# andrewhou1/BlindShadowRemoval

Hardware: AMD Instinct MI355X
Metric: images/sec at 256x256 batch inference (GSC generator forward) (higher is better)
Workload: dtype f32; 1 GPU; BASELINE configs[1]: batch=32 synthetic 256x256x3 per GPU, full GSC generator fp32 (seeded random-init weights in the ckpt-94 variable layout); global_batch=32, height=256, width=256, parallelism=dp1, forwards_in_flight=1, collective=none

## Files before the change

### blindshadowremoval_amd/csrc/bsr_api.hip

```cpp
#include "../../include/bsr_hip.h"

#include <hip/hip_runtime.h>
#include <stdint.h>
#include <stdio.h>
#include <stdlib.h>
#include <string.h>

#include <initializer_list>
#include <string>
#include <type_traits>
#include <unordered_map>
#include <vector>

#include "attention.h"
#include "attention256.h"
#include "attention_h16.h"
#include "conv3_f16.h"
#include "conv_n16.h"
#include "gemm_nloop.h"
#include "glue_kernels.h"
#include "igemm_conv.h"
#include "igemm_h16.h"
#include "png_kernels.h"
#include "prep_kernels.h"
// ... 123 lines not shown
constexpr Variant kTSM16{true, false, 291, 320, 288, 291, 320, 877, 896, 874};
constexpr Variant kRGB{false, true, 99, 128, 96, 513, 544, 0, 0, 0, 256, 3, 192, 256, 544, 128, 32};
constexpr int CS_Y3X = kGSC.cs_y3x;
constexpr int CS_CF = 64;
constexpr int RGB_CS_R = kRGB.cs_r, RGB_CS_A = kRGB.cs_a, RGB_D = kRGB.d, RGB_CS_C3 = kRGB.cs_c3, RGB_CS_C2 = kRGB.cs_c2, RGB_CS_QH = kRGB.cs_qh;

struct Region {
  size_t off, floats;
};
struct Plan {
  size_t x1, c3, c2, xa, t1, t2, y3[6], qkv, att[6], r[6], xh, ybuf, qh, f1, f2, cf, probe, reg32, share, yh, con, total;
  Region zero[8];
  int nzero;
};

Plan make_plan(size_t B, size_t H, size_t W, const Variant& v) {
  Plan p{};
  size_t off = 0;
  auto take = [&](size_t floats, bool keep_zero = false) {
    size_t o = off;
    off += (floats + 63) & ~size_t(63);
    if (keep_zero && floats != 0) p.zero[p.nzero++] = {o, floats};
    return o;
  };
  const size_t px = B * H * W, cells = px / 64;
  const size_t px2 = v.rgb ? 0 : px;
  const size_t px1 = px - px2;
  p.x1 = take(px * 32);
  p.c3 = take(px / 4 * v.cs_c3);
  p.c2 = take(px / 16 * v.cs_c2);
  p.xa = take(cells * v.cs_a, true);
  p.t1 = take(cells * v.d);
  p.t2 = take(cells * v.d);
  for (int i = 0; i < v.nblk; ++i) p.y3[i] = take(cells * v.cs_y3x);
  p.qkv = take(cells * 3 * v.d);
  for (int i = 0; i < v.nblk; ++i) p.att[i] = take(cells * v.d);
  for (int i = 0; i < v.nblk; ++i) p.r[i] = take(cells * (i < 3 ? v.cs_r : v.cs_h), !v.rgb);
  p.xh = take(cells * v.cs_h, true);
  p.ybuf = take(px * v.cs_y);
  p.qh = take(px * v.cs_qh);
  p.f1 = take(px2 / 16 * 128);
  p.f2 = take(px2 / 4 * 96);
  p.cf = take(px2 * CS_CF);
  p.probe = take(px2 / 64 * 2);
  p.reg32 = take(v.tsm ? cells * 4 : 0);
  p.share = take(v.tsm ? cells * 2 * v.c_r : 0);
  p.yh = take(px1 * 3);
  p.con = take(px1 * 3);
  p.total = off;
  return p;
}

}

struct bsr_handle {
  int device = 0;
  float* d_blob = nullptr;
  float* d_wino = nullptr;
  float* d_keys = nullptr;
  float* d_values = nullptr;
  float* att_scratch = nullptr;
  size_t att_scratch_floats = 0;
  std::unordered_map<std::string, LayerW> layers;
  Variant var = kGSC;
  int dtype = BSR_DTYPE_F32;
  float head_bias[2] = {0.f, 0.f};
  const float* tail_w = nullptr;
  const float* clr_gs_w = nullptr;
  float* ws = nullptr;
  size_t ws_floats = 0;
  Plan plan{};
  const float* rgb_tail_w = nullptr;
  const float* rgb_head_b = nullptr;
  int B = 0, H = 0, W = 0;
  bool ran = false;
  bool att_in_lds = false;
  unsigned* range_flag = nullptr;
  bool fuse_heads = true;
  bool conv1_gemm = true;
  bool att_pv1 = false;
  bool conv3_f16 = true;
  bool fuse_attw = true;
  bool wino_conv2 = true;
  bool keys_conv2 = true;
  bool values_conv2 = true;
  bool att_is_o = false;
  bool timing = false;
  std::vector<hipEvent_t> ev;
  std::vector<int> ev_class;
  std::vector<std::string> ev_name;
  size_t ev_used = 0;
};

namespace {

const char* const kRangeMsg =
    "an activation exceeded the fp16 range (|x| >= 65520) in a forward of this 16-bit-mode handle: its outputs are not trustworthy "
    "(inf / NaN where the fp32 path stays finite).  Re-run those inputs on a BSR_DTYPE_F32 handle; bsr_check_range() clears the condition";

constexpr size_t kWinoFloats = 8 * 16 * 128 * 16;
void wino_filter_transform(const float* direct, float* out) {
  static const double G[4][3] = {{1.0, 0.0, 0.0}, {0.5, 0.5, 0.5}, {0.5, -0.5, 0.5}, {0.0, 0.0, 1.0}};
  for (int k = 0; k < 128; ++k)
    for (int n = 0; n < 128; ++n) {
      double t[4][3];
      for (int x = 0; x < 4; ++x)
        for (int b = 0; b < 3; ++b) {
          double acc = 0.0;
          for (int a = 0; a < 3; ++a) acc += G[x][a] * (double)direct[((size_t)((k / 32) * 9 + a * 3 + b) * 128 + n) * 36 + k % 32];
          t[x][b] = acc;
        }
      for (int x = 0; x < 4; ++x)
        for (int y = 0; y < 4; ++y) {
          double acc = 0.0;
          for (int b = 0; b < 3; ++b) acc += t[x][b] * G[y][b];
          out[((size_t)((k / 16) * 16 + 4 * x + y) * 128 + n) * 16 + k % 16] = (float)acc;
        }
    }
}

constexpr int kKeysN = 288 + 256, kKeysNPad = kKeysN + 64, kC3qNPad = 768;
constexpr size_t kKeysFloats = (size_t)4 * kKeysNPad * 36 + kKeysNPad;
void keys_compose(const float* c3q_w, const float* c3q_b, float* out_w, float* out_b) {
  auto src = [&](int k, int n) -> const float& { return c3q_w[((size_t)(k / 32) * kC3qNPad + n) * 36 + k % 32]; };
  memset(out_w, 0, (size_t)4 * kKeysNPad * 36 * sizeof(float));
  memset(out_b, 0, kKeysNPad * sizeof(float));
  for (int ch = 0; ch < 4; ++ch) {
    memcpy(out_w + (size_t)ch * kKeysNPad * 36, c3q_w + (size_t)ch * kC3qNPad * 36, (size_t)288 * 36 * sizeof(float));
    memcpy(out_w + ((size_t)ch * kKeysNPad + 416) * 36, c3q_w + ((size_t)ch * kC3qNPad + 544) * 36, (size_t)128 * 36 * sizeof(float));
  }
  memcpy(out_b, c3q_b, 288 * sizeof(float));
  memcpy(out_b + 416, c3q_b + 544, 128 * sizeof(float));
  for (int m = 0; m < 128; ++m) {
    for (int k = 0; k < 128; ++k) {
      double acc = 0.0;
      for (int c = 0; c < 128; ++c) acc += (double)src(k, 288 + c) * (double)src(m, 416 + c);
      out_w[((size_t)(k / 32) * kKeysNPad + 288 + m) * 36 + k % 32] = (float)acc;
    }
    double acc = 0.0;
    for (int c = 0; c < 128; ++c) acc += (double)c3q_b[288 + c] * (double)src(m, 416 + c);
    out_b[288 + m] = (float)acc;
  }
}

constexpr int kWNPad = 384;
constexpr int kValuesN = 288 + 128, kValuesNPad = kValuesN + 64;
constexpr int kGProbeNPad = 128 + 64;
constexpr size_t kValuesWFloats = (size_t)4 * kWNPad * 36 + kWNPad, kValuesC3qFloats = (size_t)4 * kValuesNPad * 36 + kValuesNPad,
                 kGProbeFloats = (size_t)4 * kGProbeNPad * 36 + kGProbeNPad;
constexpr size_t kValuesFloats = kValuesWFloats + kValuesC3qFloats + kGProbeFloats;
void values_compose(const float* c3q_w, const float* c3q_b, const float* w_w, const float* w_b, float* out_w, float* out_b) {
  auto wg = [&](int k, int c) -> double { return (double)c3q_w[((size_t)(k / 32) * kC3qNPad + 544 + c) * 36 + k % 32]; };
  auto ww = [&](int c, int n) -> double { return (double)w_w[((size_t)(c / 32) * kWNPad + n) * 36 + c % 32]; };
  memset(out_w, 0, (size_t)4 * kWNPad * 36 * sizeof(float));
  for (int n = 0; n < kWNPad; ++n) {
    for (int k = 0; k < 128; ++k) {
      double acc = 0.0;
      for (int c = 0; c < 128; ++c) acc += wg(k, c) * ww(c, n);
      out_w[((size_t)(k / 32) * kWNPad + n) * 36 + k % 32] = (float)acc;
    }
    double acc = (double)w_b[n];
    for (int c = 0; c < 128; ++c) acc += (double)c3q_b[544 + c] * ww(c, n);
    out_b[n] = (float)acc;
  }
}
void values_cut(const float* keys_w, const float* keys_b, const float* c3q_w, const float* c3q_b, float* v_w, float* v_b, float* g_w, float* g_b) {
// ... 136 lines not shown
    if (half_tile) {
      if constexpr (kTrunk) check(bsr::launch_igemm_conv<KH, KW, S, TR, 2, 32, 2, 2, 1, 1, CC, INB>(a, h->B, s), name);
    } else if (!h16)
      check(bsr::launch_igemm_conv<KH, KW, S, TR, 4, 32, 4, 1, 1, NI, CC, INB>(a, h->B, s), name);
    else if (nsplit == 2)
      check(bsr::launch_igemm_h16<KH, KW, S, TR, 4, 32, 4, 1, 1, NI, CCH, INB, 2>(a, h->B, s), name);
    else if constexpr (k33)
      with_io(io, [&](auto io_c) { check(bsr::launch_igemm_h16<KH, KW, S, TR, 4, 32, 4, 1, 1, NI, CCH, INB, 1, io_c.value>(a, h->B, s), name); });
    end();
  }
  bsr::ConvArgs gemm_args(const LayerW& l, const float* in, int in_cs, float* out, int out_cs, int n_store, int act) const {
    bsr::ConvArgs a{};
    a.in = in; a.in_cs = in_cs; a.out = out; a.out_cs = out_cs;
    a.w = l.w; a.bias = l.b; a.nchunk = l.nchunk; a.n_pad = l.n_pad; a.n_store = n_store; a.act = act;
    a.range_flag = h->range_flag;
    return a;
  }
  template <int NI, int NCH, int MINW = 2>
  void gemm(int cls, const char* name, const float* in, int in_cs, size_t pixels, float* out, int out_cs, int n_store, int act,
            const float* res1 = nullptr, int res1_cs = 0, int res1_c = 0,
            float* out2 = nullptr, int out2_cs = 0, int n_split = 0, int n_store1 = 0, const LayerW* image = nullptr, int out2_gap_at = 0,
            int out2_gap = 0) {
    if (rc != BSR_OK) return;
    using C = bsr::GemmNLoopCfg<NI, NCH>;
    LayerW l;
    const int tiles = (n_store + 31) / 32;
    int kNSplit = 2;
    {
      const long long mblocks = (long long)(pixels / C::BM);
      const int want = (int)((2LL * bsr::device_cu_count() + mblocks - 1) / (mblocks > 0 ? mblocks : 1));
      const int most = (tiles + NI - 1) / NI;
      kNSplit = want < 2 ? 2 : (want > most ? most : want);
#ifdef BSR_NL_NSPLIT
      kNSplit = BSR_NL_NSPLIT > most ? most : BSR_NL_NSPLIT;
#endif
    }
    if (image == nullptr) rc = find_layer(h, name, NCH, 1, 36, (tiles + NI - 1) * 32, &l);
    else if (image->nchunk == NCH && image->ldp == 36 && image->n_pad >= (tiles + NI - 1) * 32) l = *image;
    else rc = fail(BSR_ERR_ARG, std::string("layer '") + name + "': the handle's image does not fit the kernel");
    if (rc != BSR_OK) return;
    if (pixels % C::BM != 0) { rc = fail(BSR_ERR_ARG, std::string("layer '") + name + "': pixel count is not a multiple of 128"); return; }
    bsr::ConvArgs a = gemm_args(l, in, in_cs, out, out_cs, n_store, act);
    a.res1 = res1; a.res1_cs = res1_cs; a.res1_c = res1_c;
    a.out2 = out2; a.out2_cs = out2_cs; a.n_split = n_split; a.n_store1 = n_store1; a.out2_gap_at = out2_gap_at; a.out2_gap = out2_gap;
    a.out2_split = (h->dtype != BSR_DTYPE_F32 && out2 != nullptr) ? 1 : 0;
    begin(cls, name);
    if (h->dtype == BSR_DTYPE_F32)
      check(bsr::launch_gemm_nloop<NI, NCH, 0, MINW>(a, pixels, kNSplit, s), name);
    else if constexpr (MINW == 2)
      check(bsr::launch_gemm_nloop<NI, NCH, 2>(a, pixels, kNSplit, s), name);
    else
      rc = fail(BSR_ERR_ARG, std::string("layer '") + name + "': the RGB bottleneck GEMMs are fp32 only");
    end();
  }
  template <int NCH>
  void gemm_all_n(const char* name, const float* in, size_t pixels, float* out) {
    if (rc != BSR_OK) return;
    LayerW l;
    rc = find_layer(h, name, NCH, 1, 36, 128, &l);
    if (rc != BSR_OK) return;
    begin(K_CONV1, name);
    check(bsr::launch_gemm_nloop<4, NCH, 2, 1>(gemm_args(l, in, NCH * 32, out, 128, 128, 1), pixels, 1, s), name);
    end();
  }

  void stem(const float* in, int H, int W, float* out) {
    if (rc != BSR_OK) return;
    LayerW l;
    rc = find_layer(h, "conv1", 1, 7, h->dtype != BSR_DTYPE_F32 ? 36 : 28, 32, &l);
    if (rc != BSR_OK) return;
    bsr::StemArgs a{in, out, l.w, l.b, H, W, 0, 0, 0, h->range_flag};
    begin(K_CONV7, "conv1");
    with_dtype(h->dtype, [&](auto prec, auto half) { check(bsr::launch_stem7<4, prec.value, half.value>(a, h->B, s), "conv1"); });
    end();
  }

  void wino(const char* name, int i, const float* in, int H, int W, float* out, int out_cs = 128) {
    if (rc != BSR_OK) return;
    LayerW l;
    rc = find_layer(h, name, 4, 9, 36, 128, &l);
    if (rc != BSR_OK) return;
    if (H % 4 != 0 || W % 32 != 0) { rc = fail(BSR_ERR_ARG, std::string("layer '") + name + "': feature map is not a multiple of the 4x32 tile"); return; }
    begin(K_CONV3, name);
    check(bsr::launch_wino_conv2(wino_args(in, out, h->d_wino + (size_t)i * kWinoFloats, l.b, H, W, out_cs), h->B, s), name);
    end();
  }

  void conv71(const char* name, const float* in, int in_cs, int k_pad, int H, int W, float* out, int out_cs) {
    if (rc != BSR_OK) return;
    LayerW l;
    rc = find_layer(h, name, k_pad / 32, 7, 36, 32, &l);
    if (rc != BSR_OK) return;
    if (H % 4 != 0 || W % 32 != 0) { rc = fail(BSR_ERR_ARG, std::string("layer '") + name + "': image is not a multiple of the 4x32 tile"); return; }
    bsr::ConvArgs a{};
    a.in = in; a.in_cs = in_cs; a.in_coff = 0; a.H = H; a.W = W;
    a.out = out; a.out_cs = out_cs; a.out_coff = 0; a.Ho = H; a.Wo = W;
    a.w = l.w; a.bias = l.b; a.nchunk = l.nchunk; a.n_pad = l.n_pad; a.n_store = 32;
    a.pad_t = 3; a.pad_l = 0; a.act = 0;
    begin(K_CONV7, name);
    check(bsr::launch_igemm_conv<7, 1, 1, false, 4, 32, 4, 1, 1, 1, 32, 1>(a, h->B, s), name);
    end();
  }

  void heads(const float* y, int H, int W, float* qh, const float* inputs, float* gs, float* mask22, size_t npix) {
    if (rc != BSR_OK) return;
    LayerW l;
    rc = find_layer(h, "heads", 2, 7, 36, 16, &l);
    if (rc != BSR_OK) return;
    if (l.n_pad != 16) { rc = fail(BSR_ERR_BLOB, "layer 'heads' must be packed with n_pad 16"); return; }
    if (H % 8 != 0 || W % 32 != 0) { rc = fail(BSR_ERR_ARG, "layer 'heads': image is not a multiple of its tile"); return; }
    bsr::ConvN16Args a{};
    a.in = y; a.in_cs = 64; a.H = H; a.W = W; a.w = l.w; a.bias = l.b; a.out = qh; a.out_cs = 16; a.act = 0;
    a.pad_t = 3; a.pad_l = 0;
    a.inputs = inputs; a.gs_out = gs; a.mask22 = mask22; a.b_mask = h->head_bias[0]; a.b_con = h->head_bias[1];
    a.range_flag = h->range_flag;
    int resident = 0;
    check(bsr::launch_conv_n16<7, 1, false, false, 2, 0, false, true>(a, h->B, s, &resident), "heads");
    const bool fuse = rc == BSR_OK && h->fuse_heads && bsr::conv_n16_fuse_pays(h->B, H, 8, resident);
    begin(K_CONV7, "heads");
    with_dtype(h->dtype, [&](auto prec, auto half) {
      if (fuse) check(bsr::launch_conv_n16<7, 1, false, false, 2, prec.value, half.value, true>(a, h->B, s), "heads");
      else check(bsr::launch_conv_n16<7, 1, false, false, 2, prec.value, half.value>(a, h->B, s), "heads");
    });
    end();
    if (fuse) return;
    begin(K_GLUE, "heads_post");
    hipLaunchKernelGGL(bsr::heads_post_kernel, dim3((unsigned)((npix + 255) / 256)), dim3(256), 0, s, qh, inputs, h->head_bias[0], h->head_bias[1], gs,
                       mask22, W, npix);
    check(hipGetLastError(), "heads_post");
    end();
  }

  template <int KH, int KW, bool GS, bool TAIL, int RW>
  void conv16(int cls, const char* name, const float* in, int in_cs, int H, int W, float* out, int out_cs, int act, const float* gs,
              const float* inputs, float* con_rgb, float* dif, float* packed = nullptr) {
    if (rc != BSR_OK) return;
    LayerW l;
    rc = find_layer(h, name, 2, KH * KW, 36, 16, &l);
    if (rc != BSR_OK) return;
    if (l.n_pad != 16) { rc = fail(BSR_ERR_BLOB, std::string("layer '") + name + "' must be packed with n_pad 16"); return; }
    bsr::ConvN16Args a{};
    a.in = in; a.in_cs = in_cs; a.H = H; a.W = W; a.w = l.w; a.bias = l.b; a.out = out; a.out_cs = out_cs; a.act = act;
    a.pad_t = (KH - 1) / 2; a.pad_l = (KW - 1) / 2;
    a.gs = gs; a.w_gs = h->clr_gs_w; a.tail_w = h->tail_w; a.inputs = inputs; a.con_rgb = con_rgb; a.dif = dif; a.packed = packed;
    a.range_flag = h->range_flag;
    if (H % (4 * RW) != 0 || W % 32 != 0) { rc = fail(BSR_ERR_ARG, std::string("layer '") + name + "': image is not a multiple of its tile"); return; }
    begin(cls, name);
    with_dtype(h->dtype, [&](auto prec, auto half) { check(bsr::launch_conv_n16<KH, KW, GS, TAIL, RW, prec.value, half.value>(a, h->B, s), name); });
    end();
  }
};

int grow_workspace(bsr_handle* h, size_t floats, bool device_wide, hipStream_t s) {
  if (floats <= h->ws_floats) return BSR_OK;
  if (device_wide) HIP_TRY(hipDeviceSynchronize());
  else HIP_TRY(hipStreamSynchronize(s));
  if (h->ws) HIP_TRY(hipFree(h->ws));
  h->ws = nullptr;
  h->ws_floats = 0;
  HIP_TRY(hipMalloc(reinterpret_cast<void**>(&h->ws), floats * sizeof(float)));
  h->ws_floats = floats;
  h->B = 0;
  h->ran = false;
  if (device_wide) HIP_TRY(hipMemset(h->ws, 0, floats * sizeof(float)));
  else HIP_TRY(hipMemsetAsync(h->ws, 0, floats * sizeof(float), s));
  return BSR_OK;
}

int ensure_workspace(bsr_handle* h, int B, int H, int W, hipStream_t s) {
  const Plan p = make_plan(B, H, W, h->var);
  const bool fresh = p.total > h->ws_floats;
  const int rc = grow_workspace(h, p.total, false, s);
  if (rc != BSR_OK) return rc;
  if (!fresh && (B != h->B || H != h->H || W != h->W)) {
    for (int i = 0; i < p.nzero; ++i) HIP_TRY(hipMemsetAsync(h->ws + p.zero[i].off, 0, p.zero[i].floats * sizeof(float), s));
    h->ran = false;
  }
  h->plan = p;
  h->B = B; h->H = H; h->W = W;
  return BSR_OK;
}

template <typename T>
int read_records(const unsigned char* blob, size_t off, int n, hipStream_t s, std::vector<T>* out) {
  out->resize((size_t)n);
  HIP_TRY(hipMemcpyAsync(out->data(), blob + off, (size_t)n * sizeof(T), hipMemcpyDeviceToHost, s));
  HIP_TRY(hipStreamSynchronize(s));
  return BSR_OK;
}

}

extern "C" {

int bsr_abi_version(void) { return 8; }

#ifndef BSR_SRC_SHA
#define BSR_SRC_SHA "unhashed"
#endif
static const char kSrcShaTag[] = "BSR_SRC_SHA=" BSR_SRC_SHA;
const char* bsr_source_sha(void) { return kSrcShaTag + 12; }

const char* bsr_last_error(void) { return g_last_error.c_str(); }

size_t bsr_workspace_bytes(int B, int H, int W) {
  if (B <= 0 || H <= 0 || W <= 0) return 0;
  return make_plan(B, H, W, kGSC).total * sizeof(float);
}

int bsr_create(bsr_handle** out, int device, const void* packed_weights, size_t nbytes, int dtype) {
  if (out == nullptr || packed_weights == nullptr) return fail(BSR_ERR_ARG, "bsr_create: null argument");
  *out = nullptr;
  if (dtype != BSR_DTYPE_F32 && dtype != BSR_DTYPE_F16 && dtype != BSR_DTYPE_F32X3)
    return fail(BSR_ERR_ARG, "bsr_create: dtype must be BSR_DTYPE_F32, BSR_DTYPE_F16 or BSR_DTYPE_F32X3");
  if (nbytes < sizeof(BlobHeader)) return fail(BSR_ERR_BLOB, "bsr_create: blob shorter than its header");
  const uint8_t* blob = static_cast<const uint8_t*>(packed_weights);
  BlobHeader hd;
  memcpy(&hd, blob, sizeof hd);
  if (hd.magic != kBlobMagic || hd.version != kBlobVersion) return fail(BSR_ERR_BLOB, "bsr_create: bad blob magic/version");
  if ((int)hd.reserved != dtype) return fail(BSR_ERR_BLOB, "bsr_create: the blob was packed for another dtype (pack_generator(weights, dtype) must match bsr_create's dtype)");
  const size_t table_end = sizeof(BlobHeader) + (size_t)hd.n_entries * sizeof(BlobEntry);
  if (table_end > nbytes) return fail(BSR_ERR_BLOB, "bsr_create: blob entry table exceeds blob size");
  DeviceGuard guard(device);
  HIP_TRY(guard.err);
  bsr_handle* h = new bsr_handle();
  h->device = device;
  h->dtype = dtype;
  h->att_pv1 = dtype == BSR_DTYPE_F16;
  const struct { const char* env; bool* on; } switches[] = {{"BSR_FUSE_HEADS", &h->fuse_heads}, {"BSR_FUSE_ATTW", &h->fuse_attw}, {"BSR_CONV3_F16", &h->conv3_f16},
                                                            {"BSR_CONV1_GEMM", &h->conv1_gemm}, {"BSR_WINO_CONV2", &h->wino_conv2},
                                                            {"BSR_KEYS_CONV2", &h->keys_conv2}, {"BSR_VALUES_CONV2", &h->values_conv2}};
  for (const auto& sw : switches)
    if (const char* e_ = getenv(sw.env)) *sw.on = atoi(e_) != 0;
  hipError_t e = hipMalloc(reinterpret_cast<void**>(&h->d_blob), nbytes);
  if (e == hipSuccess) e = hipMemcpy(h->d_blob, blob, nbytes, hipMemcpyHostToDevice);
  if (e != hipSuccess) {
    if (h->d_blob) hipFree(h->d_blob);
    delete h;
    return fail(BSR_ERR_HIP, std::string("bsr_create: weight upload: ") + hipGetErrorString(e));
  }
  for (uint32_t i = 0; i < hd.n_entries; ++i) {
    BlobEntry en;
    memcpy(&en, blob + sizeof(BlobHeader) + (size_t)i * sizeof(BlobEntry), sizeof en);
    en.name[sizeof(en.name) - 1] = 0;
    if (en.offset % 16 != 0 || en.offset + en.nfloats * 4 > nbytes) {
      bsr_destroy(h);
      return fail(BSR_ERR_BLOB, std::string("bsr_create: entry '") + en.name + "' is out of bounds or misaligned");
    }
    std::string nm(en.name);
    const float* dptr = reinterpret_cast<const float*>(reinterpret_cast<const uint8_t*>(h->d_blob) + en.offset);
    if (nm == "heads.bias") {
      if (en.nfloats != 2) { bsr_destroy(h); return fail(BSR_ERR_BLOB, "bsr_create: heads.bias must hold 2 floats"); }
      memcpy(h->head_bias, blob + en.offset, 8);
    } else if (nm == "clr_conv1.gs") {
      if (en.nfloats != 256) { bsr_destroy(h); return fail(BSR_ERR_BLOB, "bsr_create: clr_conv1.gs must hold 16x16 floats"); }
      h->clr_gs_w = dptr;
    } else if (nm == "rgb.tail") {
      if (en.nfloats != 7 * 7 * 3 * 3 + 3) { bsr_destroy(h); return fail(BSR_ERR_BLOB, "bsr_create: rgb.tail must hold 7x7x3x3 + 3 floats"); }
      h->rgb_tail_w = dptr;
    } else if (nm == "rgb.head_bias") {
      if (en.nfloats != 3) { bsr_destroy(h); return fail(BSR_ERR_BLOB, "bsr_create: rgb.head_bias must hold 3 floats"); }
      h->rgb_head_b = dptr;
    } else if (nm == "tail.w") {
      if (en.nfloats != 16 * 16 + 16 + 48 + 3) { bsr_destroy(h); return fail(BSR_ERR_BLOB, "bsr_create: tail.w has the wrong size"); }
      h->tail_w = dptr;
    } else if (nm.size() > 2 && nm.compare(nm.size() - 2, 2, ".w") == 0) {
      LayerW& l = h->layers[nm.substr(0, nm.size() - 2)];
      l.w = dptr;
      l.nchunk = en.dims[0]; l.taps = en.dims[1]; l.n_pad = en.dims[2]; l.ldp = en.dims[3];
      if ((uint64_t)l.nchunk * l.taps * l.n_pad * l.ldp != en.nfloats) {
        bsr_destroy(h);
        return fail(BSR_ERR_BLOB, std::string("bsr_create: entry '") + en.name + "' dims do not match its size");
      }
    } else if (nm.size() > 2 && nm.compare(nm.size() - 2, 2, ".b") == 0) {
      h->layers[nm.substr(0, nm.size() - 2)].b = dptr;
    }
  }
  if (h->layers.count("rgb_head") != 0) {
    if (dtype != BSR_DTYPE_F32) {
      bsr_destroy(h);
      return fail(BSR_ERR_ARG, "bsr_create: these are RGB-baseline weights (model_RGB.py), which run in BSR_DTYPE_F32 only: BSR_DTYPE_F32X3 and BSR_DTYPE_F16 are not provided for them");
    }
    if (h->rgb_tail_w == nullptr || h->rgb_head_b == nullptr) { bsr_destroy(h); return fail(BSR_ERR_BLOB, "bsr_create: RGB blob lacks 'rgb.tail' / 'rgb.head_bias'"); }
    h->var = kRGB;
    *out = h;
    return BSR_OK;
  }
  if (h->tail_w == nullptr || h->clr_gs_w == nullptr) { bsr_destroy(h); return fail(BSR_ERR_BLOB, "bsr_create: blob lacks 'tail.w' / 'clr_conv1.gs'"); }
  if (dtype != BSR_DTYPE_F32) {
    e = hipHostMalloc(reinterpret_cast<void**>(&h->range_flag), 64, hipHostMallocMapped);
    if (e != hipSuccess) { h->range_flag = nullptr; bsr_destroy(h); return fail(BSR_ERR_HIP, std::string("bsr_create: range flag: ") + hipGetErrorString(e)); }
    *h->range_flag = 0u;
  }
  {
    auto it = h->layers.find("res0.conv1");
    if (it == h->layers.end()) { bsr_destroy(h); return fail(BSR_ERR_BLOB, "bsr_create: blob has no 'res0.conv1'"); }
    const int nch = it->second.nchunk;
    if (dtype == BSR_DTYPE_F32) h->var = nch == 13 ? kTSM : kGSC;
    else h->var = nch == 10 ? kTSM16 : kGSC16;
  }
  if (dtype == BSR_DTYPE_F32) {
    std::vector<float> u(6 * kWinoFloats);
    for (int i = 0; i < 6; ++i) {
      char nm[32];
      snprintf(nm, sizeof nm, "res%d.conv2", i);
      LayerW l;
      if (find_layer(h, nm, 4, 9, 36, 128, &l) != BSR_OK || l.n_pad != 128) { bsr_destroy(h); return fail(BSR_ERR_BLOB, std::string("bsr_create: layer '") + nm + "' is not a [4][9][128][36] image"); }
      wino_filter_transform(reinterpret_cast<const float*>(blob + (reinterpret_cast<const uint8_t*>(l.w) - reinterpret_cast<const uint8_t*>(h->d_blob))), u.data() + i * kWinoFloats);
    }
    e = hipMalloc(reinterpret_cast<void**>(&h->d_wino), u.size() * sizeof(float));
    if (e == hipSuccess) e = hipMemcpy(h->d_wino, u.data(), u.size() * sizeof(float), hipMemcpyHostToDevice);
    if (e != hipSuccess) { bsr_destroy(h); return fail(BSR_ERR_HIP, std::string("bsr_create: Winograd weights: ") + hipGetErrorString(e)); }
    std::vector<float> q(6 * kKeysFloats);
// ... 997 lines not shown
size_t bsr_sfw_score_scratch_bytes(int B, int S) { return post_size_ok(B, S) ? (size_t)B * bsr::sfw_item_scratch_bytes(S) : 0; }

int bsr_sfw_score(int device, const float* rows3, int B, int S, float* losses, double* auc, float* pred, float* label, int* status,
                  void* scratch, void* stream) {
  return run_post("bsr_sfw_score", {rows3, losses, auc, pred, label, status, scratch}, B, S, scratch, device, [&] {
    HIP_TRY(bsr::launch_sfw_score(rows3, B, S, losses, auc, pred, label, status, scratch, static_cast<hipStream_t>(stream)));
    return BSR_OK;
  });
}

int bsr_clock_trace(int device, unsigned long long* out, int samples, int spin, const int* stop, int* taken, void* stream) {
  if (out == nullptr || stop == nullptr || taken == nullptr || samples <= 0 || spin < 0) return fail(BSR_ERR_ARG, "bsr_clock_trace: bad argument");
  DeviceGuard guard(device);
  HIP_TRY(guard.err);
  hipLaunchKernelGGL(bsr::clock_trace_kernel, dim3(1), dim3(64), 0, static_cast<hipStream_t>(stream), out, samples, spin, stop, taken);
  HIP_TRY(hipGetLastError());
  return BSR_OK;
}

int bsr_debug_split_qkv(const float* qkv, void* qkv_split, int B, int tokens, void* stream) {
  if (qkv == nullptr || qkv_split == nullptr) return fail(BSR_ERR_ARG, "bsr_debug_split_qkv: null argument");
  if (B <= 0 || tokens <= 0 || tokens % 128 != 0) return fail(BSR_ERR_ARG, "bsr_debug_split_qkv: tokens must be a positive multiple of 128");
  const size_t pairs = (size_t)B * tokens * 192;
  hipLaunchKernelGGL(bsr::a4_split_qkv_kernel, dim3((unsigned)((pairs + 255) / 256)), dim3(256), 0, static_cast<hipStream_t>(stream), qkv,
                     static_cast<char*>(qkv_split), pairs);
  HIP_TRY(hipGetLastError());
  return BSR_OK;
}

int bsr_debug_attention_split(const void* qkv_split, float* y, int B, int tokens, int pv1, void* stream) {
  if (qkv_split == nullptr || y == nullptr) return fail(BSR_ERR_ARG, "bsr_debug_attention_split: null argument");
  if (B <= 0 || tokens <= 0 || tokens % 128 != 0) return fail(BSR_ERR_ARG, "bsr_debug_attention_split: tokens must be a positive multiple of 128");
  HIP_TRY(bsr::launch_nonlocal_attention_h16(static_cast<const float*>(qkv_split), y, B, tokens, static_cast<hipStream_t>(stream), pv1 != 0));
  return BSR_OK;
}

int bsr_debug_attention_dtype(const float* qkv, float* y, int B, int tokens, int dtype, void* stream) {
  if (qkv == nullptr || y == nullptr) return fail(BSR_ERR_ARG, "bsr_debug_attention: null argument");
  if (B <= 0 || tokens <= 0 || tokens % 128 != 0) return fail(BSR_ERR_ARG, "bsr_debug_attention: tokens must be a positive multiple of 128");
  if (dtype == BSR_DTYPE_F32) {
    HIP_TRY(bsr::launch_nonlocal_attention(qkv, y, B, tokens, static_cast<hipStream_t>(stream)));
  } else if (dtype == BSR_DTYPE_F32X3 || dtype == BSR_DTYPE_F16) {
    void* tmp = nullptr;
    HIP_TRY(hipMalloc(&tmp, (size_t)B * tokens * bsr::kA4TokBytes));
    int rc = bsr_debug_split_qkv(qkv, tmp, B, tokens, stream);
    if (rc == BSR_OK) rc = bsr_debug_attention_split(tmp, y, B, tokens, 0, stream);
    hipError_t e = hipStreamSynchronize(static_cast<hipStream_t>(stream));
    hipFree(tmp);
    if (rc != BSR_OK) return rc;
    HIP_TRY(e);
  } else {
    return fail(BSR_ERR_ARG, "bsr_debug_attention: unknown dtype");
  }
  return BSR_OK;
}

int bsr_debug_attention_qw(const float* qkv, float* y, int B, int tokens, int qw, void* stream) {
  if (qkv == nullptr || y == nullptr) return fail(BSR_ERR_ARG, "bsr_debug_attention_qw: null argument");
  if (B <= 0 || tokens <= 0 || tokens % 128 != 0) return fail(BSR_ERR_ARG, "bsr_debug_attention_qw: tokens must be a positive multiple of 128");
  if (qw != 0 && qw != 1 && qw != 2 && qw != 4) return fail(BSR_ERR_ARG, "bsr_debug_attention_qw: qw must be 0 (automatic), 1, 2 or 4 query waves per workgroup");
  HIP_TRY(bsr::launch_nonlocal_attention(qkv, y, B, tokens, static_cast<hipStream_t>(stream), qw));
  return BSR_OK;
}

int bsr_debug_attention_kv1(const float* qkv2, float* y, int B, int tokens, int qw, void* stream) {
  if (qkv2 == nullptr || y == nullptr) return fail(BSR_ERR_ARG, "bsr_debug_attention_kv1: null argument");
  if (B <= 0 || tokens <= 0 || tokens % 128 != 0) return fail(BSR_ERR_ARG, "bsr_debug_attention_kv1: tokens must be a positive multiple of 128");
  if (qw != 0 && qw != 1 && qw != 2 && qw != 4) return fail(BSR_ERR_ARG, "bsr_debug_attention_kv1: qw must be 0 (automatic), 1, 2 or 4 query waves per workgroup");
  HIP_TRY(bsr::launch_nonlocal_attention<true>(qkv2, y, B, tokens, static_cast<hipStream_t>(stream), qw));
  return BSR_OK;
}

int bsr_debug_attention_rgb(const float* qkv, float* y, int B, int tokens, void* stream) {
  if (qkv == nullptr || y == nullptr) return fail(BSR_ERR_ARG, "bsr_debug_attention_rgb: null argument");
  if (B <= 0 || tokens <= 0 || tokens % 32 != 0) return fail(BSR_ERR_ARG, "bsr_debug_attention_rgb: tokens must be a positive multiple of 32");
  HIP_TRY(bsr::launch_nonlocal_attention256(qkv, y, B, tokens, static_cast<hipStream_t>(stream)));
  return BSR_OK;
}

int bsr_debug_wino_conv(const float* x, const float* w, const float* bias, float* y, int B, int H, int W, int nw, void* stream) {
  if (x == nullptr || w == nullptr || bias == nullptr || y == nullptr) return fail(BSR_ERR_ARG, "bsr_debug_wino_conv: null argument");
  if (B <= 0 || H <= 0 || W <= 0 || H % 4 != 0 || W % 32 != 0) return fail(BSR_ERR_ARG, "bsr_debug_wino_conv: H must be a positive multiple of 4 and W of 32");
  if ((long long)B * H * W * 128 * 4 >= (1LL << 31)) return fail(BSR_ERR_ARG, "bsr_debug_wino_conv: tensor too large");
  if (nw != 0 && nw != 2 && nw != 4) return fail(BSR_ERR_ARG, "bsr_debug_wino_conv: nw must be 0 (automatic), 2 or 4 waves per workgroup");
  HIP_TRY(bsr::launch_wino_conv2(wino_args(x, y, w, bias, H, W), B, static_cast<hipStream_t>(stream), nw));
  return BSR_OK;
}

int bsr_debug_wino_filter(const float* direct, float* out) {
  if (direct == nullptr || out == nullptr) return fail(BSR_ERR_ARG, "bsr_debug_wino_filter: null argument");
  wino_filter_transform(direct, out);
  return BSR_OK;
}

int bsr_debug_keys_compose(const float* c3q_w, const float* c3q_b, float* out_w, float* out_b) {
  if (c3q_w == nullptr || c3q_b == nullptr || out_w == nullptr || out_b == nullptr) return fail(BSR_ERR_ARG, "bsr_debug_keys_compose: null argument");
  keys_compose(c3q_w, c3q_b, out_w, out_b);
  return BSR_OK;
}

int bsr_debug_values_compose(const float* c3q_w, const float* c3q_b, const float* w_w, const float* w_b, float* out_w, float* out_b) {
  if (c3q_w == nullptr || c3q_b == nullptr || w_w == nullptr || w_b == nullptr || out_w == nullptr || out_b == nullptr)
    return fail(BSR_ERR_ARG, "bsr_debug_values_compose: null argument");
  values_compose(c3q_w, c3q_b, w_w, w_b, out_w, out_b);
  return BSR_OK;
}

int bsr_debug_attention(const float* qkv, float* y, int B, int tokens, void* stream) {
  return bsr_debug_attention_dtype(qkv, y, B, tokens, BSR_DTYPE_F32, stream);
}

struct ProbeSrc { size_t off; int hh, ww, cs, coff, c; bool half; int derive; };

static int probe_index(const std::string& nm, const char* prefix, int n) {
  const size_t len = strlen(prefix);
  if (nm.size() == len + 1 && nm.compare(0, len, prefix) == 0 && nm[len] >= '0' && nm[len] < '0' + n) return nm[len] - '0';
  return -1;
}

static int probe_src_rgb(const bsr_handle* h, const std::string& nm, ProbeSrc* src) {
  const Plan& p = h->plan;
  const int H = h->H, W = h->W;
  int i;
  if (nm == "x1") *src = {p.x1, H, W, 32, 0, 32};
  else if (nm == "x2") *src = {p.c3, H / 2, W / 2, RGB_CS_C3, 128, 64};
  else if (nm == "x3") *src = {p.c2, H / 4, W / 4, RGB_CS_C2, 192, 64};
  else if (nm == "x0") *src = {p.xa, H / 8, W / 8, RGB_CS_A, 0, 99};
  else if ((i = probe_index(nm, "res", 3)) >= 0) *src = {p.r[i], H / 8, W / 8, RGB_CS_R, 0, 513};
  else if ((i = probe_index(nm, "att", 3)) >= 0) *src = {p.att[i], H / 8, W / 8, RGB_D, 0, RGB_D};
  else if ((i = probe_index(nm, "y3x", 3)) >= 0) *src = {p.y3[i], H / 8, W / 8, RGB_CS_R, 0, 513};
  else if (nm == "up1") *src = {p.c2, H / 4, W / 4, RGB_CS_C2, 0, 192};
  else if (nm == "up2") *src = {p.c3, H / 2, W / 2, RGB_CS_C3, 0, 128};
  else if (nm == "up3") *src = {p.ybuf, H, W, 128, 0, 128};
  else if (nm == "y") *src = {p.yh, H, W, 3, 0, 3};
  else if (nm == "con") *src = {p.con, H, W, 3, 0, 3};
  else return fail(BSR_ERR_STATE, "bsr_probe: unknown probe '" + nm + "' for an RGB handle");
  return BSR_OK;
}

static int probe_src_gsc(const bsr_handle* h, const std::string& nm, ProbeSrc* src) {
  const Plan& p = h->plan;
  const Variant& v = h->var;
  const int H = h->H, W = h->W;
  const bool p16 = h->dtype == BSR_DTYPE_F16;
  int i;
  if (nm == "x1") *src = {p.x1, H, W, 32, 0, 32, p16};
  else if (nm == "x2") *src = {p.c3, H / 2, W / 2, 128, 64, 64, p16};
  else if (nm == "x3") *src = {p.c2, H / 4, W / 4, 160, 96, 64, p16};
  else if (nm == "x0") *src = {p.xa, H / 8, W / 8, v.cs_a, 0, v.c_a};
  else if ((i = probe_index(nm, "res", 6)) >= 0) *src = {p.r[i], H / 8, W / 8, i < 3 ? v.cs_r : v.cs_h, 0, i < 3 ? v.c_r : v.c_h};
  else if ((i = probe_index(nm, "att", 6)) >= 0) {
    if (h->att_in_lds)
      return fail(BSR_ERR_STATE, "bsr_probe: att<i> does not exist for the last forward — attention and the `w` GEMM ran as one launch and the "
                                 "attention output never left LDS (create the handle with BSR_FUSE_ATTW=0 in the environment to probe it)");
    *src = {p.att[i], H / 8, W / 8, 128, 0, 128, false, h->att_is_o ? i + 1 : 0};
  }
  else if ((i = probe_index(nm, "attv", 6)) >= 0) {
    if (!h->att_is_o) return fail(BSR_ERR_STATE, "bsr_probe: attv<i> exists only for a forward with conv2's output as the attention values (fp32, BSR_KEYS_CONV2 and BSR_VALUES_CONV2 on)");
    if (h->att_in_lds)
      return fail(BSR_ERR_STATE, "bsr_probe: attv<i> does not exist for the last forward — attention and the `w` GEMM ran as one launch and the "
                                 "attention output never left LDS (create the handle with BSR_FUSE_ATTW=0 in the environment to probe it)");
    *src = {p.att[i], H / 8, W / 8, 128, 0, 128};
  }
  else if (nm == "qkv") {
    if (h->dtype != BSR_DTYPE_F32) return fail(BSR_ERR_STATE, "bsr_probe: qkv is an fp32 tensor of BSR_DTYPE_F32 handles only");
    const int c = h->att_is_o ? 256 : 384;
    *src = {p.qkv, H / 8, W / 8, c, 0, c};
// ... 95 lines not shown
```

### blindshadowremoval_amd/csrc/wino_conv2.h

```cpp
#pragma once
#include <hip/hip_runtime.h>
#include <stdint.h>

#include "mfma_common.h"

namespace bsr {

struct WinoArgs {
  const float* in;
  float* out;
  const float* w;
  const float* bias;
  int H, W;
  int in_cs, out_cs;
  int tiles_x, tiles_y;
  int act;
};

template <int NW>
struct WinoCfg {
  static constexpr int NT = NW * 64;
  static constexpr int CC = 16;
  static constexpr int LDP = CC + 4;
  static constexpr int K = 128, N = 128, NCHUNK = K / CC;
// ... 121 lines not shown
  for (int i = 0; i < 4; ++i) store_w1(u_n1, w_regs[1], i);
  fetch_w(2, w_regs[1]);
  __syncthreads();

  f32x16 acc[16];
#pragma unroll
  for (int q = 0; q < 16; ++q)
#pragma unroll
    for (int i = 0; i < 16; ++i) acc[q][i] = 0.f;
  acc[5] = bias_tile(h, bias_n);

  const int a_base = r * LDP + 4 * h;
  const int b_base = (wave * 32 + r) * LDP + 4 * h;
  f32x4 af[2], bf[2];
  auto read_frags = [&](int slot, int v_off, int u_off) {
    af[slot] = *reinterpret_cast<const f32x4*>(s_v + a_base + v_off);
    bf[slot] = *reinterpret_cast<const f32x4*>(s_u + b_base + u_off);
  };
  read_frags(0, v_cur, u_cur);

  for (int ch = 0; ch < C::NCHUNK; ++ch) {
    const int ch1 = ch + 1 < C::NCHUNK ? ch + 1 : C::NCHUNK - 1;
#pragma unroll
    for (int s = 0; s < SPC; ++s) {
      const int t = ch * SPC + s;
      fetch_w(t + 3 < NSTEPS ? t + 3 : NSTEPS - 1, w_regs[s & 1]);
      if (s == 0) fetch_in(ch1, d);
      __builtin_amdgcn_sched_barrier(0);
#pragma unroll
      for (int q = 0; q < 4; ++q) {
        const int cur = q & 1, nxt = cur ^ 1;
        const int pl = q >> 1;
        if (q < 3) {
          const int pl1 = (q + 1) >> 1, g1 = (q + 1) & 1;
          read_frags(nxt, v_cur + (2 * s + pl1) * C::V_POS + g1 * 8, u_cur + pl1 * C::U_POS + g1 * 8);
        } else if (s + 1 < SPC) {
          read_frags(nxt, v_cur + (2 * s + 2) * C::V_POS, u_n1);
        } else {
          read_frags(nxt, v_nxt, u_n1);
        }
        store_w1(u_n2, w_regs[(s + 1) & 1], q);
        if (s == SPC - 3) in_rows(d, q);
        if (s == SPC - 2) in_cols_store(v_nxt, d, q);
        __builtin_amdgcn_sched_barrier(0);
#pragma unroll
        for (int j = 0; j < 4; ++j)
          acc[2 * s + pl] = __builtin_amdgcn_mfma_f32_32x32x2f32(af[cur][j], bf[cur][j], acc[2 * s + pl], 0, 0, 0);
        __builtin_amdgcn_sched_barrier(0);
      }
      __syncthreads();
      { const int tu = u_cur; u_cur = u_n1; u_n1 = u_n2; u_n2 = tu; }
      if (s == SPC - 1) { const int tv = v_cur; v_cur = v_nxt; v_nxt = tv; }
    }
  }

  const float alpha = p.act ? kLeakyAlpha : 1.f;
  const unsigned cs4 = (unsigned)p.out_cs * 4u;
  const __amdgpu_buffer_rsrc_t orsrc =
      make_rsrc(p.out + ((size_t)img * p.H * p.W + (size_t)y0 * p.W + x0) * p.out_cs + n0 + wave * 32);
  const unsigned lane_out = (unsigned)(8 * h) * cs4 + (unsigned)r * 4u;
#pragma unroll
  for (int v = 0; v < 16; ++v) {
    float t0[4], t1[4];
#pragma unroll
    for (int nu = 0; nu < 4; ++nu) {
      t0[nu] = (acc[nu][v] + acc[4 + nu][v]) + acc[8 + nu][v];
      t1[nu] = (acc[4 + nu][v] - acc[8 + nu][v]) - acc[12 + nu][v];
    }
    f32x2 y0v = f32x2{(t0[0] + t0[1]) + t0[2], (t0[1] - t0[2]) - t0[3]};
    f32x2 y1v = f32x2{(t1[0] + t1[1]) + t1[2], (t1[1] - t1[2]) - t1[3]};
    const f32x2 s0 = y0v * alpha, s1 = y1v * alpha;
    const int prow = 2 * (v >> 3), pcol = 2 * (8 * ((v >> 2) & 1) + (v & 3));
#pragma unroll
    for (int i = 0; i < 2; ++i)
#pragma unroll
      for (int j = 0; j < 2; ++j) {
        const float x = i ? y1v[j] : y0v[j], ax = i ? s1[j] : s0[j];
        const unsigned soff = (unsigned)((prow + i) * p.W + pcol + j) * cs4;
        __builtin_amdgcn_raw_buffer_store_b32(__float_as_uint(__builtin_amdgcn_fmed3f(x, ax, 3.4028234664e38f)), orsrc, lane_out, soff, 0);
      }
  }
}

inline int wino_conv2_auto_nw(int batch, int H, int W) {
  const long long tiles = (long long)batch * (H / 4) * (W / 32);
  return 2 * tiles <= device_cu_count() ? 2 : 4;
}

template <int NW>
inline hipError_t launch_wino_conv2_nw(WinoArgs a, int batch, hipStream_t stream) {
  using C = WinoCfg<NW>;
  auto kern = wino_conv2_kernel<NW>;
  static PerDeviceOnce once;
  const int dev = PerDeviceOnce::current();
  if (dev < 0 || !once.done[dev]) {
    hipError_t e = hipFuncSetAttribute(reinterpret_cast<const void*>(kern), hipFuncAttributeMaxDynamicSharedMemorySize, C::SMEM_BYTES);
    if (e != hipSuccess) return e;
    if (dev >= 0) once.done[dev] = true;
  }
  a.tiles_x = a.W / 32;
  a.tiles_y = a.H / 4;
  dim3 grid(a.tiles_x * a.tiles_y * batch, 4 / NW);
  hipLaunchKernelGGL(kern, grid, dim3(C::NT), C::SMEM_BYTES, stream, a);
  return hipGetLastError();
}

inline hipError_t launch_wino_conv2(const WinoArgs& a, int batch, hipStream_t stream, int nw = 0) {
  if (nw == 0) nw = wino_conv2_auto_nw(batch, a.H, a.W);
  return nw == 2 ? launch_wino_conv2_nw<2>(a, batch, stream) : launch_wino_conv2_nw<4>(a, batch, stream);
}

}
```

Baseline: 7012 images/sec.

## Add 8-wave Winograd conv kernel splitting transform positions across wave pairs

Adds a 512-thread Winograd F(2x2,3x3) conv kernel in which two groups of four waves each handle half of the 16 transform positions for the same output tile. The groups exchange partial output-transform sums through LDS before storing. Weights are triple-buffered in LDS and the next input chunk is fetched while MFMAs run. This is meant to raise per-CU concurrency and latency hiding on the wino conv layers, at the cost of an extra LDS exchange and a larger LDS footprint per block. It is on by default whenever the auto heuristic would pick 4 waves.

Result: faster. 7089 images/sec (median of 6 runs) (+1.1%).

```diff
diff --git a/blindshadowremoval_amd/csrc/bsr_api.hip b/blindshadowremoval_amd/csrc/bsr_api.hip
--- a/blindshadowremoval_amd/csrc/bsr_api.hip
+++ b/blindshadowremoval_amd/csrc/bsr_api.hip
@@ -229,6 +229,7 @@
   bool conv3_f16 = true;
   bool fuse_attw = true;
   bool wino_conv2 = true;
+  bool wino_pairs = true;
   bool keys_conv2 = true;
   bool values_conv2 = true;
   bool att_is_o = false;
@@ -531,7 +532,7 @@
     if (rc != BSR_OK) return;
     if (H % 4 != 0 || W % 32 != 0) { rc = fail(BSR_ERR_ARG, std::string("layer '") + name + "': feature map is not a multiple of the 4x32 tile"); return; }
     begin(K_CONV3, name);
-    check(bsr::launch_wino_conv2(wino_args(in, out, h->d_wino + (size_t)i * kWinoFloats, l.b, H, W, out_cs), h->B, s), name);
+    check(bsr::launch_wino_conv2(wino_args(in, out, h->d_wino + (size_t)i * kWinoFloats, l.b, H, W, out_cs), h->B, s, 0, h->wino_pairs), name);
     end();
   }
 
@@ -677,7 +678,7 @@
   h->dtype = dtype;
   h->att_pv1 = dtype == BSR_DTYPE_F16;
   const struct { const char* env; bool* on; } switches[] = {{"BSR_FUSE_HEADS", &h->fuse_heads}, {"BSR_FUSE_ATTW", &h->fuse_attw}, {"BSR_CONV3_F16", &h->conv3_f16},
-                                                            {"BSR_CONV1_GEMM", &h->conv1_gemm}, {"BSR_WINO_CONV2", &h->wino_conv2},
+                                                            {"BSR_CONV1_GEMM", &h->conv1_gemm}, {"BSR_WINO_CONV2", &h->wino_conv2}, {"BSR_WINO_PAIRS", &h->wino_pairs},
                                                             {"BSR_KEYS_CONV2", &h->keys_conv2}, {"BSR_VALUES_CONV2", &h->values_conv2}};
   for (const auto& sw : switches)
     if (const char* e_ = getenv(sw.env)) *sw.on = atoi(e_) != 0;
@@ -1841,7 +1842,7 @@
   if (x == nullptr || w == nullptr || bias == nullptr || y == nullptr) return fail(BSR_ERR_ARG, "bsr_debug_wino_conv: null argument");
   if (B <= 0 || H <= 0 || W <= 0 || H % 4 != 0 || W % 32 != 0) return fail(BSR_ERR_ARG, "bsr_debug_wino_conv: H must be a positive multiple of 4 and W of 32");
   if ((long long)B * H * W * 128 * 4 >= (1LL << 31)) return fail(BSR_ERR_ARG, "bsr_debug_wino_conv: tensor too large");
-  if (nw != 0 && nw != 2 && nw != 4) return fail(BSR_ERR_ARG, "bsr_debug_wino_conv: nw must be 0 (automatic), 2 or 4 waves per workgroup");
+  if (nw != 0 && nw != 2 && nw != 4 && nw != 8) return fail(BSR_ERR_ARG, "bsr_debug_wino_conv: nw must be 0 (automatic), 2, 4 or 8 waves per workgroup");
   HIP_TRY(bsr::launch_wino_conv2(wino_args(x, y, w, bias, H, W), B, static_cast<hipStream_t>(stream), nw));
   return BSR_OK;
 }
diff --git a/blindshadowremoval_amd/csrc/wino_conv2.h b/blindshadowremoval_amd/csrc/wino_conv2.h
--- a/blindshadowremoval_amd/csrc/wino_conv2.h
+++ b/blindshadowremoval_amd/csrc/wino_conv2.h
@@ -227,9 +227,231 @@
   }
 }
 
+struct WinoPairCfg {
+  static constexpr int NT = 512;
+  static constexpr int CC = 16, LDP = CC + 4;
+  static constexpr int K = 128, N = 128, NCHUNK = K / CC;
+  static constexpr int SPC = 4;
+  static constexpr int NSTEPS = NCHUNK * SPC;
+  static constexpr int V_POS = 32 * LDP;
+  static constexpr int V_FLOATS = 16 * V_POS;
+  static constexpr int U_POS = N * LDP;
+  static constexpr int U_FLOATS = 4 * U_POS;
+  static constexpr int SMEM_BYTES = (V_FLOATS + 3 * U_FLOATS) * 4;
+  static constexpr int X_FLOATS = 8 * 32 * 64;
+  static_assert(SMEM_BYTES <= 160 * 1024 && X_FLOATS * 4 <= SMEM_BYTES, "LDS budget");
+};
+
+__global__ __launch_bounds__(512, 2) void wino_conv2_pairs_kernel(WinoArgs p) {
+  using C = WinoPairCfg;
+  constexpr int LDP = C::LDP, SPC = C::SPC, NSTEPS = C::NSTEPS;
+  typedef unsigned u32x4_t __attribute__((ext_vector_type(4)));
+  extern __shared__ __attribute__((aligned(16))) float smem[];
+  float* s_v = smem;
+  float* s_u = smem + C::V_FLOATS;
+
+  const int tid = threadIdx.x;
+  const int lane = tid & 63;
+  const int wave = __builtin_amdgcn_readfirstlane(tid >> 6);
+  const int wq = wave & 3, c = wave >> 2;
+  const int h = lane >> 5, r = lane & 31;
+
+  int bid = blockIdx.x;
+  const int tile_x = bid % p.tiles_x;
+  bid /= p.tiles_x;
+  const int tile_y = bid % p.tiles_y;
+  const int img = bid / p.tiles_y;
+  const int y0 = tile_y * 4, x0 = tile_x * 32;
+  const float* in_img = p.in + (size_t)img * p.H * p.W * p.in_cs;
+  const __amdgpu_buffer_rsrc_t in_rsrc = make_rsrc(in_img);
+
+  unsigned in_goff[16];
+  const int patch = tid >> 4, cn = tid & 15;
+  {
+    const int py = patch >> 4, px = patch & 15;
+#pragma unroll
+    for (int a = 0; a < 4; ++a)
+#pragma unroll
+      for (int b = 0; b < 4; ++b) {
+        const int iy = y0 + 2 * py - 1 + a, ix = x0 + 2 * px - 1 + b;
+        const bool ok = iy >= 0 && iy < p.H && ix >= 0 && ix < p.W;
+        in_goff[4 * a + b] = ok ? (unsigned)(((iy * p.W + ix) * p.in_cs + cn) * 4) : kLaneOff;
+      }
+  }
+  const int v_loff = patch * LDP + cn;
+  const unsigned w_goff = (unsigned)(tid * 16);
+  const int w_loff = (tid >> 2) * LDP + (tid & 3) * 4;
+  const __amdgpu_buffer_rsrc_t w_rsrc = make_rsrc(p.w);
+  constexpr unsigned kPosBytes = (unsigned)(C::N * C::CC * 4);
+  const float bias_n = c == 0 ? p.bias[wq * 32 + r] : 0.f;
+
+  auto fetch_in = [&](int chunk, float (&d)[16]) {
+    const unsigned soff = (unsigned)(chunk * C::CC * 4);
+#pragma unroll
+    for (int i = 0; i < 16; ++i)
+      d[i] = __uint_as_float(__builtin_amdgcn_raw_buffer_load_b32(in_rsrc, in_goff[i], soff, 0));
+  };
+  auto in_rows = [&](float (&d)[16], int b) {
+    const float d0 = d[b], d1 = d[4 + b], d2 = d[8 + b], d3 = d[12 + b];
+    d[b] = d0 - d2;
+    d[4 + b] = d1 + d2;
+    d[8 + b] = d2 - d1;
+    d[12 + b] = d1 - d3;
+  };
+  auto in_cols_store = [&](const float (&d)[16], int a) {
+    const float w0 = d[4 * a], w1 = d[4 * a + 1], w2 = d[4 * a + 2], w3 = d[4 * a + 3];
+    float* dst = s_v + v_loff + 4 * a * C::V_POS;
+    dst[0] = w0 - w2;
+    dst[C::V_POS] = w1 + w2;
+    dst[2 * C::V_POS] = w2 - w1;
+    dst[3 * C::V_POS] = w1 - w3;
+  };
+  auto fetch_w1 = [&](int t, f32x4 (&regs)[4], int j) {
+    regs[j] = __builtin_bit_cast(f32x4, (u32x4_t)__builtin_amdgcn_raw_buffer_load_b128(w_rsrc, w_goff, (unsigned)(4 * t + j) * kPosBytes, 0));
+  };
+  auto store_w1 = [&](int u_off, const f32x4 (&regs)[4], int i) {
+    *reinterpret_cast<f32x4*>(s_u + u_off + i * C::U_POS + w_loff) = regs[i];
+  };
+
+  float d[16];
+  f32x4 w_regs[4];
+  int u_cur = 0, u_n1 = C::U_FLOATS, u_n2 = 2 * C::U_FLOATS;
+  fetch_in(0, d);
+#pragma unroll
+  for (int t = 0; t < 2; ++t) {
+#pragma unroll
+    for (int i = 0; i < 4; ++i) fetch_w1(t, w_regs, i);
+#pragma unroll
+    for (int i = 0; i < 4; ++i) store_w1(t * C::U_FLOATS, w_regs, i);
+  }
+#pragma unroll
+  for (int i = 0; i < 4; ++i) fetch_w1(2, w_regs, i);
+#pragma unroll
+  for (int b = 0; b < 4; ++b) in_rows(d, b);
+#pragma unroll
+  for (int a = 0; a < 3; ++a) in_cols_store(d, a);
+  __syncthreads();
+
+  f32x16 acc[8];
+#pragma unroll
+  for (int q = 0; q < 8; ++q)
+#pragma unroll
+    for (int i = 0; i < 16; ++i) acc[q][i] = 0.f;
+  acc[3] = bias_tile(h, bias_n);
+
+  const int a_base = 2 * c * C::V_POS + r * LDP + 4 * h;
+  const int b_base = 2 * c * C::U_POS + (wq * 32 + r) * LDP + 4 * h;
+  f32x4 af[2], bf[2];
+  auto read_frags = [&](int slot, int v_off, int u_off) {
+    af[slot] = *reinterpret_cast<const f32x4*>(s_v + a_base + v_off);
+    bf[slot] = *reinterpret_cast<const f32x4*>(s_u + b_base + u_off);
+  };
+  read_frags(0, 0, u_cur);
+
+  if (c) __builtin_amdgcn_s_setprio(1);
+#pragma unroll 1
+  for (int ch = 0; ch < C::NCHUNK; ++ch) {
+    const int ch1 = ch + 1 < C::NCHUNK ? ch + 1 : C::NCHUNK - 1;
+#pragma unroll
+    for (int s = 0; s < SPC; ++s) {
+      const int t = ch * SPC + s;
+      const int t3 = t + 3 < NSTEPS ? t + 3 : NSTEPS - 1;
+#pragma unroll
+      for (int q = 0; q < 4; ++q) {
+        const int cur = q & 1, nxt = cur ^ 1;
+        const int pl = q >> 1;
+        if (q < 3) {
+          const int pl1 = (q + 1) >> 1, g1 = (q + 1) & 1;
+          read_frags(nxt, (4 * s + pl1) * C::V_POS + g1 * 8, u_cur + pl1 * C::U_POS + g1 * 8);
+        } else {
+          read_frags(nxt, (4 * ((s + 1) % SPC)) * C::V_POS, u_n1);
+        }
+        store_w1(u_n2, w_regs, q);
+        fetch_w1(t3, w_regs, q);
+        if (s == 0 && q == 0) in_cols_store(d, 3);
+        if (s == 0 && q == 1) fetch_in(ch1, d);
+        if (s == 2 && q == 0) { in_rows(d, 0); in_rows(d, 1); }
+        if (s == 2 && q == 1) { in_rows(d, 2); in_rows(d, 3); }
+        if (s == 2 && q == 2) in_cols_store(d, 0);
+        if (s == 2 && q == 3) in_cols_store(d, 1);
+        if (s == 3 && q == 0) in_cols_store(d, 2);
+        __builtin_amdgcn_sched_barrier(0);
+#pragma unroll
+        for (int j = 0; j < 4; ++j)
+          acc[2 * s + pl] = __builtin_amdgcn_mfma_f32_32x32x2f32(af[cur][j], bf[cur][j], acc[2 * s + pl], 0, 0, 0);
+        __builtin_amdgcn_sched_barrier(0);
+      }
+      __syncthreads();
+      { const int tu = u_cur; u_cur = u_n1; u_n1 = u_n2; u_n2 = tu; }
+    }
+  }
+
+  __builtin_amdgcn_s_setprio(0);
+  float t0[2][16], t1[2][16];
+#pragma unroll
+  for (int pl = 0; pl < 2; ++pl)
+#pragma unroll
+    for (int v = 0; v < 16; ++v) {
+      t0[pl][v] = (acc[pl][v] + acc[2 + pl][v]) + acc[4 + pl][v];
+      t1[pl][v] = (acc[2 + pl][v] - acc[4 + pl][v]) - acc[6 + pl][v];
+    }
+  float* x_mine = smem + (wave * 32) * 64 + lane;
+  const float* x_theirs = smem + ((wave ^ 4) * 32) * 64 + lane;
+#pragma unroll
+  for (int v = 0; v < 16; ++v) {
+    x_mine[v * 64] = c ? t0[0][v] : t0[1][v];
+    x_mine[(16 + v) * 64] = c ? t1[0][v] : t1[1][v];
+  }
+  __syncthreads();
+  float y0v[16], y1v[16];
+  if (c == 0) {
+#pragma unroll
+    for (int v = 0; v < 16; ++v) {
+      y0v[v] = (t0[0][v] + t0[1][v]) + x_theirs[v * 64];
+      y1v[v] = (t1[0][v] + t1[1][v]) + x_theirs[(16 + v) * 64];
+    }
+  } else {
+#pragma unroll
+    for (int v = 0; v < 16; ++v) {
+      y0v[v] = (x_theirs[v * 64] - t0[0][v]) - t0[1][v];
+      y1v[v] = (x_theirs[(16 + v) * 64] - t1[0][v]) - t1[1][v];
+    }
+  }
+  const float alpha = p.act ? kLeakyAlpha : 1.f;
+  const unsigned cs4 = (unsigned)p.out_cs * 4u;
+  const __amdgpu_buffer_rsrc_t orsrc =
+      make_rsrc(p.out + ((size_t)img * p.H * p.W + (size_t)y0 * p.W + x0) * p.out_cs + wq * 32);
+  const unsigned lane_out = (unsigned)(8 * h) * cs4 + (unsigned)r * 4u;
+#pragma unroll
+  for (int v = 0; v < 16; ++v) {
+    const int prow = 2 * (v >> 3), pcol = 2 * (8 * ((v >> 2) & 1) + (v & 3));
+#pragma unroll
+    for (int i = 0; i < 2; ++i) {
+      const float x = i ? y1v[v] : y0v[v];
+      const unsigned soff = (unsigned)((prow + i) * p.W + pcol + c) * cs4;
+      __builtin_amdgcn_raw_buffer_store_b32(__float_as_uint(__builtin_amdgcn_fmed3f(x, x * alpha, 3.4028234664e38f)), orsrc, lane_out, soff, 0);
+    }
+  }
+}
+
 inline int wino_conv2_auto_nw(int batch, int H, int W) {
   const long long tiles = (long long)batch * (H / 4) * (W / 32);
   return 2 * tiles <= device_cu_count() ? 2 : 4;
+}
+
+inline hipError_t launch_wino_conv2_pairs(WinoArgs a, int batch, hipStream_t stream) {
+  using C = WinoPairCfg;
+  static PerDeviceOnce once;
+  const int dev = PerDeviceOnce::current();
+  if (dev < 0 || !once.done[dev]) {
+    hipError_t e = hipFuncSetAttribute(reinterpret_cast<const void*>(wino_conv2_pairs_kernel), hipFuncAttributeMaxDynamicSharedMemorySize, C::SMEM_BYTES);
+    if (e != hipSuccess) return e;
+    if (dev >= 0) once.done[dev] = true;
+  }
+  a.tiles_x = a.W / 32;
+  a.tiles_y = a.H / 4;
+  hipLaunchKernelGGL(wino_conv2_pairs_kernel, dim3(a.tiles_x * a.tiles_y * batch), dim3(C::NT), C::SMEM_BYTES, stream, a);
+  return hipGetLastError();
 }
 
 template <int NW>
@@ -250,8 +472,12 @@
   return hipGetLastError();
 }
 
-inline hipError_t launch_wino_conv2(const WinoArgs& a, int batch, hipStream_t stream, int nw = 0) {
-  if (nw == 0) nw = wino_conv2_auto_nw(batch, a.H, a.W);
+inline hipError_t launch_wino_conv2(const WinoArgs& a, int batch, hipStream_t stream, int nw = 0, bool pairs = true) {
+  if (nw == 0) {
+    nw = wino_conv2_auto_nw(batch, a.H, a.W);
+    if (nw == 4 && pairs) nw = 8;
+  }
+  if (nw == 8) return launch_wino_conv2_pairs(a, batch, stream);
   return nw == 2 ? launch_wino_conv2_nw<2>(a, batch, stream) : launch_wino_conv2_nw<4>(a, batch, stream);
 }
 
```
